# angelocatalani/neural-network-compression

Hardware: AMD Instinct MI355X
Metric: weights/sec through prune+k-means (K=256) (higher is better)
Workload: dtype f32

## Files before the change

### neural_network_compression_amd/csrc/nnc_sort.hip

```cpp
#include <hip/hip_runtime.h>
#include <cmath>
#include <cstdlib>
#include <cstring>

#include <algorithm>
#include <string>

#include "nnc.h"

extern "C" const char *nnc_last_error(void);
int nnc_set_error_(int code, const char *msg);

#ifndef OS_THREADS
#define OS_THREADS 1024
#endif
#define OS_WAVES (OS_THREADS / 64)
#ifndef OS_ITEMS
#define OS_ITEMS 16
#endif
#ifndef OS_BLOCKS_PER_CU
#define OS_BLOCKS_PER_CU 1
#endif
#ifndef OS_RANK_LDS
#define OS_RANK_LDS 1
#endif
#define OS_TILE (OS_THREADS * OS_ITEMS)
#define OS_MAXBITS 9
#define OS_MAXR (1 << OS_MAXBITS)
#define OS_MAXPASS 4
#define OS_SPIN_LIMIT (1 << 22)
#define OSP_THREADS 1024
#define OSP_PER 16
#define OSP_TILE (OSP_THREADS * OSP_PER)

__device__ __forceinline__ unsigned f32_ord(float v)
{
    const unsigned b = __float_as_uint(v);
    return (b & 0x80000000u) ? ~b : (b | 0x80000000u);
}
__device__ __forceinline__ float f32_unord(unsigned o)
{
    return __uint_as_float((o & 0x80000000u) ? (o ^ 0x80000000u) : ~o);
}

struct OsMap { unsigned lo_neg, hi_neg, lo_pos, hi_pos, span_neg; int bounded; };
struct OsPlan { int passes; int shift[OS_MAXPASS]; int rb[OS_MAXPASS]; };

__device__ __forceinline__ unsigned os_key(const OsMap &m, float e, bool &outside)
{
    const unsigned o = f32_ord(e);
    if (!m.bounded) return o;
    if (e < 0.0f) { outside |= (o < m.lo_neg) | (o > m.hi_neg); const unsigned c = o < m.lo_neg ? m.lo_neg : (o > m.hi_neg ? m.hi_neg : o); return c - m.lo_neg; }
    outside |= (o < m.lo_pos) | (o > m.hi_pos);
    const unsigned c = o < m.lo_pos ? m.lo_pos : (o > m.hi_pos ? m.hi_pos : o);
    return m.span_neg + (c - m.lo_pos);
}
__device__ __forceinline__ float os_value(const OsMap &m, unsigned k)
{
    if (!m.bounded) return f32_unord(k);
    return f32_unord(k < m.span_neg ? k + m.lo_neg : k - m.span_neg + m.lo_pos);
}

#define OS_CTRL_WORDS 4

template <bool SKIPZ>
__global__ __launch_bounds__(OSP_THREADS) void k_os_prep(const float *__restrict__ x, long long n, unsigned *__restrict__ keys,
                                                         unsigned long long *__restrict__ ctrl, long long cap, OsMap km, int rb0, unsigned *__restrict__ ghist)
{
    __shared__ unsigned comp_s[SKIPZ ? OSP_TILE : 1];
    __shared__ unsigned hist_s[OS_MAXR];
    __shared__ unsigned wave_tot[OSP_THREADS / 64];
    __shared__ unsigned long long base_s;
    const int tid = threadIdx.x, lane = tid & 63, wv = tid >> 6;
    for (int i = tid; i < OS_MAXR; i += OSP_THREADS) hist_s[i] = 0u;
    __syncthreads();
    const bool vec = (reinterpret_cast<uintptr_t>(x) & 15) == 0;
    const float4 *x4 = reinterpret_cast<const float4 *>(x);
    const unsigned mask0 = (1u << rb0) - 1u;
    bool outside = false;
    const long long ntiles = (n + OSP_TILE - 1) / OSP_TILE;
    auto load_tile = [&](long long tt, float (&e)[OSP_PER]) {
        const long long tile0 = tt * OSP_TILE;
        if (tt >= ntiles) return;
        if (vec && tile0 + OSP_TILE <= n) {
#pragma unroll
            for (int j = 0; j < OSP_PER / 4; j++) {
                const float4 q = x4[(tile0 >> 2) + (long long)j * OSP_THREADS + tid];
                e[4 * j] = q.x; e[4 * j + 1] = q.y; e[4 * j + 2] = q.z; e[4 * j + 3] = q.w;
            }
        } else {
#pragma unroll
            for (int j = 0; j < OSP_PER; j++) {
                const long long i = tile0 + (long long)j * OSP_THREADS + tid;
                e[j] = i < n ? x[i] : 0.0f;
            }
        }
    };
    float en[OSP_PER];
    load_tile(blockIdx.x, en);
    for (long long t = blockIdx.x; t < ntiles; t += gridDim.x) {
        const long long tile0 = t * OSP_TILE;
        const bool fast = vec && tile0 + OSP_TILE <= n;
        float e[OSP_PER];
#pragma unroll
        for (int j = 0; j < OSP_PER; j++) e[j] = en[j];
        load_tile(t + gridDim.x, en);
        unsigned key[OSP_PER];
        unsigned take = 0;
#pragma unroll
        for (int j = 0; j < OSP_PER; j++) {
            bool ok = SKIPZ ? !(e[j] == 0.0f) : true;
            if (!SKIPZ && !fast) ok = tile0 + (long long)j * OSP_THREADS + tid < n;
            key[j] = 0u;
            if (ok) { key[j] = os_key(km, e[j], outside); take |= 1u << j; }
        }
#pragma unroll
        for (int j = 0; j < OSP_PER; j++)
            if (take & (1u << j)) atomicAdd(&hist_s[key[j] & mask0], 1u);
        if (SKIPZ) {
            const unsigned c = (unsigned)__popc(take);
            unsigned sc = c;
            for (int off = 1; off < 64; off <<= 1) { const unsigned o = __shfl_up(sc, off); if (lane >= off) sc += o; }
            if (lane == 63) wave_tot[wv] = sc;
            __syncthreads();
            unsigned pre = 0, tot = 0;
            for (int w = 0; w < OSP_THREADS / 64; w++) { const unsigned o = wave_tot[w]; if (w < wv) pre += o; tot += o; }
            if (tid == 0) base_s = atomicAdd(ctrl, (unsigned long long)tot);
            unsigned at = pre + sc - c;
#pragma unroll
            for (int j = 0; j < OSP_PER; j++)
                if (take & (1u << j)) comp_s[at++] = key[j];
            __syncthreads();
            const long long base = (long long)base_s;
            for (unsigned i = tid; i < tot; i += OSP_THREADS)
                if (base + i < cap) keys[base + i] = comp_s[i];
            __syncthreads();
        }
    }
    if (outside) atomicOr(ctrl + 1, 1ull);
    __syncthreads();
    for (int i = tid; i < OS_MAXR; i += OSP_THREADS) {
        const unsigned v = hist_s[i];
        if (v) atomicAdd(&ghist[i], v);
    }
}

#ifdef NNC_DIAG
__device__ unsigned long long *g_os_trace = nullptr;
extern "C" int nnc_debug_os_trace(void *buf)
{
    unsigned long long *p = reinterpret_cast<unsigned long long *>(buf);
    return hipMemcpyToSymbol(HIP_SYMBOL(g_os_trace), &p, sizeof(p)) == hipSuccess ? NNC_OK : NNC_EHIP;
}
#define OS_STAMP(i) do { if (g_os_trace && t == 0) g_os_trace[((size_t)pass * 8192 + (size_t)(tile < 8192 ? tile : 8191)) * 8 + (i)] = __builtin_amdgcn_s_memrealtime(); } while (0)
#else
#define OS_STAMP(i) do { } while (0)
#endif

__device__ __forceinline__ void os_publish(unsigned long long *w, unsigned tag, unsigned v)
{
    __hip_atomic_store(w, ((unsigned long long)tag << 32) | v, __ATOMIC_RELAXED, __HIP_MEMORY_SCOPE_AGENT);
}
__device__ __forceinline__ unsigned long long os_peek(const unsigned long long *w)
{
    return __hip_atomic_load(w, __ATOMIC_RELAXED, __HIP_MEMORY_SCOPE_AGENT);
}

template <int RB, bool FULL>
__device__ __forceinline__ void os_peers(unsigned d, bool valid, unsigned &plo, unsigned &phi)
{
    const unsigned long long all = FULL ? ~0ull : __ballot(valid);
    plo = (unsigned)all; phi = (unsigned)(all >> 32);
#pragma unroll
    for (int b = 0; b < RB; b++) {
        const int m = ((int)(d << (31 - b))) >> 31;
        const unsigned long long mb = FULL ? __ballot(m != 0) : __ballot(valid && m != 0);
        plo &= ~((unsigned)mb ^ (unsigned)m);
        phi &= ~((unsigned)(mb >> 32) ^ (unsigned)m);
    }
}

#ifndef OS_LOOK
#define OS_LOOK 4
#endif

template <int RB, int SRC, int DST>
__global__ __launch_bounds__(OS_THREADS, OS_BLOCKS_PER_CU * OS_THREADS / 256) void k_os_pass(const void *__restrict__ in_, void *__restrict__ out_, long long n, int shift, int pass, int nrb,
                                                           const unsigned *__restrict__ ghist, unsigned *__restrict__ ghist_next, unsigned long long *__restrict__ status,
                                                           unsigned long long *__restrict__ ctrl, OsMap km, long long n_neg, long long n_zero, int abl)
{
    constexpr int R = 1 << RB;
    constexpr unsigned MASK = (unsigned)R - 1u;
    constexpr int DPT = (R + OS_THREADS - 1) / OS_THREADS;
    __shared__ unsigned keys_s[OS_TILE];
    __shared__ unsigned short wcnt[OS_WAVES][R];
    __shared__ unsigned short tpre[R];
    __shared__ unsigned gpos[R];
    __shared__ unsigned gdig[R];
    __shared__ unsigned nhist[OS_MAXR];
    __shared__ unsigned wsum[OS_WAVES];
    __shared__ long long tile_s;
    const int t = threadIdx.x, lane = t & 63, wv = t >> 6;
    const unsigned *in_k = reinterpret_cast<const unsigned *>(in_);
    const float *in_f = reinterpret_cast<const float *>(in_);
    unsigned *out_k = reinterpret_cast<unsigned *>(out_);
    float *out_f = reinterpret_cast<float *>(out_);
    const unsigned tagA = 2u * (unsigned)pass + 1u, tagP = tagA + 1u;
    unsigned *ticket = reinterpret_cast<unsigned *>(ctrl + 2) + pass;
    const int nshift = shift + RB;
    const unsigned nmask = nrb > 0 ? (1u << nrb) - 1u : 0u;
    {
        unsigned v[DPT], own = 0;
#pragma unroll
        for (int r = 0; r < DPT; r++) { const int d = t * DPT + r; v[r] = d < R ? ghist[d] : 0u; own += v[r]; }
        unsigned sc = own;
        for (int off = 1; off < 64; off <<= 1) { const unsigned o = __shfl_up(sc, off); if (lane >= off) sc += o; }
        if (lane == 63) wsum[wv] = sc;
        for (int i = t; i < OS_MAXR; i += OS_THREADS) nhist[i] = 0u;
        __syncthreads();
        unsigned run = sc - own;
        for (int w = 0; w < wv; w++) run += wsum[w];
#pragma unroll
        for (int r = 0; r < DPT; r++) { const int d = t * DPT + r; if (d < R) gdig[d] = run; run += v[r]; }
        __syncthreads();
    }
    const long long ntiles = (n + OS_TILE - 1) / OS_TILE;
    bool gave_up = false;
    for (;;) {
        if (t == 0) tile_s = (long long)atomicAdd(ticket, 1u);
        for (int d = t; d < R; d += OS_THREADS) {
#pragma unroll
            for (int w = 0; w < OS_WAVES; w++) wcnt[w][d] = 0;
        }
#if OS_RANK_LDS
        static_assert((size_t)OS_WAVES * R * 8 <= (size_t)OS_TILE * 4, "lane masks do not fit the tile buffer");
        for (int i = t; i < OS_WAVES * R * 2; i += OS_THREADS) keys_s[i] = 0u;
#endif
        __syncthreads();
        const long long tile = tile_s;
        if (tile >= ntiles) break;
        OS_STAMP(0);
        const long long tile0 = tile * OS_TILE;
        const int cnt_tile = (int)((n - tile0) < OS_TILE ? (n - tile0) : OS_TILE);
        const bool full = cnt_tile == OS_TILE;
        unsigned key[OS_ITEMS];
        unsigned short rnk[OS_ITEMS];
#pragma unroll
        for (int i = 0; i < OS_ITEMS; i++) {
            const int idx = wv * (64 * OS_ITEMS) + i * 64 + lane;
            if (SRC == 0) key[i] = (full || idx < cnt_tile) ? in_k[tile0 + idx] : 0xFFFFFFFFu;
            else key[i] = (full || idx < cnt_tile) ? f32_ord(in_f[tile0 + idx]) : 0xFFFFFFFFu;
        }
#ifdef NNC_DIAG
        if (g_os_trace) { if (key[OS_ITEMS - 1] == 0x12345678u && key[0] == 0x87654321u) keys_s[0] = 1u; OS_STAMP(1); }
#endif
        if (nrb > 0) {
#pragma unroll
            for (int i = 0; i < OS_ITEMS; i++) {
                const int idx = wv * (64 * OS_ITEMS) + i * 64 + lane;
                if ((full || idx < cnt_tile) && !(abl & 8)) atomicAdd(&nhist[(key[i] >> nshift) & nmask], 1u);
            }
        }
#pragma unroll
        for (int i = 0; i < OS_ITEMS; i++) {
            const int idx = wv * (64 * OS_ITEMS) + i * 64 + lane;
            const bool valid = full || idx < cnt_tile;
            const unsigned d = (key[i] >> shift) & MASK;
            unsigned plo, phi;
#if OS_RANK_LDS
            unsigned long long *mrow = reinterpret_cast<unsigned long long *>(keys_s) + wv * R;
            if (valid) atomicOr(&mrow[d], 1ull << lane);
            __builtin_amdgcn_wave_barrier();
            const unsigned long long pm = valid ? mrow[d] : 0ull;
            plo = (unsigned)pm; phi = (unsigned)(pm >> 32);
            if (abl & 2) { plo = lane < 32 ? 1u << lane : 0u; phi = lane >= 32 ? 1u << (lane - 32) : 0u; }
#else
            if (abl & 2) { plo = lane < 32 ? 1u << lane : 0u; phi = lane >= 32 ? 1u << (lane - 32) : 0u; }
            else if (full) os_peers<RB, true>(d, true, plo, phi);
            else os_peers<RB, false>(d, valid, plo, phi);
#endif
            const unsigned before = (unsigned)__builtin_amdgcn_mbcnt_hi(phi, __builtin_amdgcn_mbcnt_lo(plo, 0u));
            unsigned prev = 0;
            if (valid) {
                prev = wcnt[wv][d];
                if (before == 0) {
                    wcnt[wv][d] = (unsigned short)(prev + (unsigned)__popc(plo) + (unsigned)__popc(phi));
#if OS_RANK_LDS
                    mrow[d] = 0ull;
#endif
                }
            }
            rnk[i] = (unsigned short)(prev + before);
            __builtin_amdgcn_wave_barrier();
        }
        __syncthreads();
        OS_STAMP(2);
        unsigned tc[DPT], own = 0;
#pragma unroll
        for (int r = 0; r < DPT; r++) {
            const int d = t * DPT + r;
            tc[r] = 0;
            if (d < R) {
                unsigned run = 0;
#pragma unroll
                for (int w = 0; w < OS_WAVES; w++) { const unsigned c = wcnt[w][d]; wcnt[w][d] = (unsigned short)run; run += c; }
                tc[r] = run;
                os_publish(&status[(size_t)tile * R + d], tile == 0 ? tagP : tagA, run);
            }
            own += tc[r];
        }
        {
            unsigned sc = own;
            for (int off = 1; off < 64; off <<= 1) { const unsigned o = __shfl_up(sc, off); if (lane >= off) sc += o; }
            if (lane == 63) wsum[wv] = sc;
            __syncthreads();
            unsigned run = sc - own;
            for (int w = 0; w < wv; w++) run += wsum[w];
#pragma unroll
            for (int r = 0; r < DPT; r++) { const int d = t * DPT + r; if (d < R) tpre[d] = (unsigned short)run; run += tc[r]; }
        }
        __syncthreads();
#pragma unroll
        for (int i = 0; i < OS_ITEMS; i++) {
            const int idx = wv * (64 * OS_ITEMS) + i * 64 + lane;
            if (full || idx < cnt_tile) {
                const unsigned d = (key[i] >> shift) & MASK;
                keys_s[(unsigned)tpre[d] + (unsigned)wcnt[wv][d] + (unsigned)rnk[i]] = key[i];
            }
        }
        OS_STAMP(3);
        if (DST == 1 && n_zero > 0) {
            const long long per = ((n_zero + ntiles - 1) / ntiles + 3) & ~3ll;
            const long long z0 = tile * per, z1 = (z0 + per < n_zero) ? z0 + per : n_zero;
            float *zp = out_f + n_neg;
            if ((reinterpret_cast<uintptr_t>(zp) & 15) == 0) {
                for (long long i = z0 + 4ll * t; i + 3 < z1; i += 4ll * OS_THREADS) *reinterpret_cast<float4 *>(zp + i) = make_float4(0.f, 0.f, 0.f, 0.f);
                if (t == 0) for (long long i = z0 + ((z1 - z0) & ~3ll); i < z1; i++) zp[i] = 0.0f;
            } else {
                for (long long i = z0 + t; i < z1; i += OS_THREADS) zp[i] = 0.0f;
            }
        }
#pragma unroll
        for (int r = 0; r < DPT; r++) {
            const int d = t * DPT + r;
            if (d >= R) continue;
            unsigned excl = 0;
            if (tile > 0 && !(abl & 1)) {
                long long i = tile - 1;
                int polls = 0;
                bool done = false;
                while (!done) {
                    unsigned long long w[OS_LOOK];
#pragma unroll
                    for (int j = 0; j < OS_LOOK; j++) w[j] = (i - j >= 0) ? os_peek(&status[(size_t)(i - j) * R + d]) : 0ull;
                    int used = 0;
#pragma unroll
                    for (int j = 0; j < OS_LOOK; j++) {
                        if (!done && used == j) {
                            const unsigned tg = (unsigned)(w[j] >> 32);
                            if (tg == tagP) { excl += (unsigned)w[j]; done = true; }
                            else if (tg == tagA) { excl += (unsigned)w[j]; used = j + 1; }
                        }
                    }
                    if (!done) {
                        i -= used;
                        if (used == 0) {
                            if (++polls > OS_SPIN_LIMIT) { gave_up = true; done = true; }
                            __builtin_amdgcn_s_sleep(1);
                        } else polls = 0;
                    }
                }
                os_publish(&status[(size_t)tile * R + d], tagP, excl + tc[r]);
            }
            gpos[d] = gdig[d] + excl - (unsigned)tpre[d];
        }
        OS_STAMP(4);
        __syncthreads();
        OS_STAMP(5);
        for (int j = t; j < cnt_tile; j += OS_THREADS) {
            const unsigned kv = keys_s[j];
            const unsigned d = (kv >> shift) & MASK;
            const unsigned r = gpos[d] + (unsigned)j;
            if ((long long)r < n && !(abl & 4)) {
                if (DST == 0) out_k[r] = kv;
                else out_f[(long long)r + ((long long)r >= n_neg ? n_zero : 0)] = os_value(km, kv);
            }
        }
        OS_STAMP(6);
        __syncthreads();
        OS_STAMP(7);
    }
    if (gave_up) atomicOr(ctrl + 1, 2ull);
    if (nrb > 0) {
        for (int i = t; i <= (int)nmask; i += OS_THREADS) {
            const unsigned v = nhist[i];
            if (v) atomicAdd(&ghist_next[i], v);
        }
    }
}

static unsigned host_ord(float v)
{
    unsigned b;
    std::memcpy(&b, &v, 4);
    return (b & 0x80000000u) ? ~b : (b | 0x80000000u);
}

static size_t al256(size_t b) { return (b + 255) & ~(size_t)255; }

static int os_cus()
{
    static int cus[64] = {0};
    int dev = 0;
    if (hipGetDevice(&dev) != hipSuccess || dev < 0 || dev >= 64) return 256;
    if (!cus[dev]) {
        int v = 0;
        if (hipDeviceGetAttribute(&v, hipDeviceAttributeMultiprocessorCount, dev) != hipSuccess || v <= 0) v = 256;
        cus[dev] = v;
    }
    return cus[dev];
}

static OsPlan os_plan(int bits)
{
    OsPlan pl;
    std::memset(&pl, 0, sizeof(pl));
    int rb;
    if (bits <= 8) { pl.passes = 1; rb = 8; }
    else if (bits <= 16) { pl.passes = 2; rb = 8; }
    else if (bits <= 18) { pl.passes = 2; rb = 9; }
    else if (bits <= 24) { pl.passes = 3; rb = 8; }
    else if (bits <= 27) { pl.passes = 3; rb = 9; }
    else { pl.passes = 4; rb = 8; }
    for (int p = 0; p < pl.passes; p++) { pl.shift[p] = p * rb; pl.rb[p] = rb; }
    return pl;
}

static size_t os_status_bytes(int64_t n_keys)
{
    const int64_t ntiles = (n_keys + OS_TILE - 1) / OS_TILE;
    return al256((size_t)std::max<int64_t>(ntiles, 1) * OS_MAXR * 8);
}
static size_t os_ws_bytes(int64_t n_keys)
{
    return 2 * al256((size_t)n_keys * 4 + 16) + al256(OS_CTRL_WORDS * 8) + al256((size_t)(OS_MAXPASS + 1) * OS_MAXR * 4) + os_status_bytes(n_keys) + 256;
}
static unsigned char *os_ws_base(void *ws) { return reinterpret_cast<unsigned char *>((reinterpret_cast<uintptr_t>(ws) + 255) & ~(uintptr_t)255); }

static int os_sort(const float *x, int64_t n, bool skip_zeros, int64_t n_neg, int64_t n_zero, const OsMap &km, int bits, float *sorted_out, void *ws,
                   size_t ws_bytes, int32_t *flag_dev, const char *who, void *stream)
{
    const int64_t n_keys = skip_zeros ? n - n_zero : n;
    if (!ws || ws_bytes < os_ws_bytes(n_keys)) return nnc_set_error_(NNC_ENOSPACE, (std::string(who) + ": workspace too small").c_str());
    hipStream_t s = reinterpret_cast<hipStream_t>(stream);
    unsigned char *b = os_ws_base(ws);
    unsigned *ka = reinterpret_cast<unsigned *>(b); b += al256((size_t)n_keys * 4 + 16);
    unsigned *kb = reinterpret_cast<unsigned *>(b); b += al256((size_t)n_keys * 4 + 16);
    unsigned long long *ctrl = reinterpret_cast<unsigned long long *>(b); b += al256(OS_CTRL_WORDS * 8);
    unsigned *ghist = reinterpret_cast<unsigned *>(b); b += al256((size_t)(OS_MAXPASS + 1) * OS_MAXR * 4);
    unsigned long long *status = reinterpret_cast<unsigned long long *>(b);
    hipError_t e;
    const size_t zero_bytes = al256(OS_CTRL_WORDS * 8) + al256((size_t)(OS_MAXPASS + 1) * OS_MAXR * 4) + os_status_bytes(n_keys);
    if ((e = hipMemsetAsync(ctrl, 0, zero_bytes, s)) != hipSuccess) return nnc_set_error_(NNC_EHIP, hipGetErrorString(e));
    if (skip_zeros && n_zero > 0 && n_keys == 0 && (e = hipMemsetAsync(sorted_out + n_neg, 0, (size_t)n_zero * 4, s)) != hipSuccess) return nnc_set_error_(NNC_EHIP, hipGetErrorString(e));
    const OsPlan pl = os_plan(bits);
    int abl = 0;
#ifdef NNC_DIAG
    { const char *ev = getenv("NNC_OS_ABLATE"); abl = ev ? atoi(ev) : 0; }
#endif
    if (n_keys > 0) {
        const long long ptiles = (n + OSP_TILE - 1) / OSP_TILE;
        const int pgrid = (int)std::min<long long>(std::max<long long>(ptiles, 1), 2LL * os_cus());
        if (skip_zeros) hipLaunchKernelGGL((k_os_prep<true>), dim3(pgrid), dim3(OSP_THREADS), 0, s, x, (long long)n, ka, ctrl, (long long)n_keys, km, pl.rb[0], ghist);
        else hipLaunchKernelGGL((k_os_prep<false>), dim3(pgrid), dim3(OSP_THREADS), 0, s, x, (long long)n, (unsigned *)nullptr, ctrl, (long long)n_keys, km, pl.rb[0], ghist);
        if ((e = hipGetLastError()) != hipSuccess) return nnc_set_error_(NNC_EHIP, hipGetErrorString(e));
        const long long ntiles = (n_keys + OS_TILE - 1) / OS_TILE;
        const int grid = (int)std::min<long long>(ntiles, (long long)OS_BLOCKS_PER_CU * os_cus());
        const void *src = skip_zeros ? (const void *)ka : (const void *)x;
        unsigned *dst = skip_zeros ? kb : ka;
        for (int p = 0; p < pl.passes; p++) {
            const bool first_f = (p == 0 && !skip_zeros), last = (p == pl.passes - 1);
            void *o = last ? (void *)sorted_out : (void *)dst;
#define OS_LAUNCH(SRC, DST) do { \
                if (pl.rb[p] == 9) hipLaunchKernelGGL((k_os_pass<9, SRC, DST>), dim3(grid), dim3(OS_THREADS), 0, s, src, o, (long long)n_keys, pl.shift[p], p, last ? 0 : pl.rb[p + 1], \
                                                      ghist + (size_t)p * OS_MAXR, ghist + (size_t)(p + 1) * OS_MAXR, status, ctrl, km, (long long)(skip_zeros ? n_neg : n_keys), (long long)(skip_zeros ? n_zero : 0), abl); \
                else hipLaunchKernelGGL((k_os_pass<8, SRC, DST>), dim3(grid), dim3(OS_THREADS), 0, s, src, o, (long long)n_keys, pl.shift[p], p, last ? 0 : pl.rb[p + 1], \
                                        ghist + (size_t)p * OS_MAXR, ghist + (size_t)(p + 1) * OS_MAXR, status, ctrl, km, (long long)(skip_zeros ? n_neg : n_keys), (long long)(skip_zeros ? n_zero : 0), abl); \
            } while (0)
            if (first_f && last) OS_LAUNCH(1, 1);
            else if (first_f) OS_LAUNCH(1, 0);
            else if (last) OS_LAUNCH(0, 1);
            else OS_LAUNCH(0, 0);
#undef OS_LAUNCH
            if ((e = hipGetLastError()) != hipSuccess) return nnc_set_error_(NNC_EHIP, hipGetErrorString(e));
            src = dst;
            dst = (dst == ka) ? kb : ka;
        }
    }
    if (flag_dev && (e = hipMemcpyAsync(flag_dev, reinterpret_cast<unsigned char *>(ctrl) + 8, 4, hipMemcpyDeviceToDevice, s)) != hipSuccess)
        return nnc_set_error_(NNC_EHIP, hipGetErrorString(e));
    return NNC_OK;
}

static OsMap os_identity()
{
    OsMap m;
    std::memset(&m, 0, sizeof(m));
    return m;
}

extern "C" size_t nnc_sort_workspace_bytes(int64_t n) { return n <= 0 ? 0 : os_ws_bytes(n); }

extern "C" int nnc_sort_f32(const float *x, int64_t n, float *sorted_out, void *ws, size_t ws_bytes, void *stream)
{
    if (n < 0 || n >= ((int64_t)1 << 31) || (n > 0 && (!x || !sorted_out))) return nnc_set_error_(NNC_EINVAL, "nnc_sort_f32: bad argument");
    if (n == 0) return NNC_OK;
    return os_sort(x, n, false, 0, 0, os_identity(), 32, sorted_out, ws, ws_bytes, nullptr, "nnc_sort_f32", stream);
}

extern "C" size_t nnc_sort_pruned_workspace_bytes(int64_t n, int64_t n_neg, int64_t n_zero)
{
    if (n <= 0 || n_neg < 0 || n_zero < 0 || n_neg + n_zero > n) return 0;
    return os_ws_bytes(n - n_zero);
}

extern "C" int nnc_sort_pruned_f32(const float *x, int64_t n, int64_t n_neg, int64_t n_zero, float *sorted_out, void *ws,
                                   size_t ws_bytes, void *stream)
{
    if (n < 0 || n_neg < 0 || n_zero < 0 || n_neg + n_zero > n || n >= ((int64_t)1 << 31) || (n > 0 && (!x || !sorted_out)))
        return nnc_set_error_(NNC_EINVAL, "nnc_sort_pruned_f32: bad argument");
    if (n == 0) return NNC_OK;
    return os_sort(x, n, true, n_neg, n_zero, os_identity(), 32, sorted_out, ws, ws_bytes, nullptr, "nnc_sort_pruned_f32", stream);
}

static int rs_bounds(float vmin, float vmax, float thr, int64_t n_neg, int64_t n_pos, OsMap *bd)
{
    if (!(thr > 0.0f) || !std::isfinite(thr) || !std::isfinite(vmin) || !std::isfinite(vmax)) return 0;
    OsMap b;
    std::memset(&b, 0, sizeof(b));
    b.bounded = 1;
    unsigned long long total = 0;
    if (n_neg > 0) {
        if (!(vmin <= -thr)) return 0;
        b.lo_neg = host_ord(vmin); b.hi_neg = host_ord(-thr);
        b.span_neg = b.hi_neg - b.lo_neg + 1u;
        total += b.span_neg;
    }
    if (n_pos > 0) {
        if (!(vmax >= thr)) return 0;
        b.lo_pos = host_ord(thr); b.hi_pos = host_ord(vmax);
        total += (unsigned long long)(b.hi_pos - b.lo_pos) + 1ull;
    }
    if (total == 0 || total > (1ull << 27)) return 0;
    int bits = 1;
    while ((1ull << bits) < total) bits++;
    *bd = b;
    return bits;
}

extern "C" int32_t nnc_sort_pruned_bounded_bits(float vmin, float vmax, float thr, int64_t n_neg, int64_t n_pos)
{
    OsMap b;
    return rs_bounds(vmin, vmax, thr, n_neg, n_pos, &b);
}

extern "C" size_t nnc_sort_pruned_bounded_workspace_bytes(int64_t n_nz)
{
    if (n_nz < 0) return 0;
    return os_ws_bytes(n_nz);
}

int nnc_sort_pruned_bounded_flagged_(const float *x, int64_t n, int64_t n_neg, int64_t n_zero, float vmin, float vmax, float thr,
                                     float *sorted_out, void *ws, size_t ws_bytes, int32_t *flag_dev, void *stream);
extern "C" int nnc_sort_pruned_bounded_f32(const float *x, int64_t n, int64_t n_neg, int64_t n_zero, float vmin, float vmax, float thr,
                                           float *sorted_out, void *ws, size_t ws_bytes, void *stream)
{
    return nnc_sort_pruned_bounded_flagged_(x, n, n_neg, n_zero, vmin, vmax, thr, sorted_out, ws, ws_bytes, nullptr, stream);
}

extern "C" const int32_t *nnc_sort_pruned_bounded_flag(void *ws, int64_t n_nonzero)
{
    if (!ws || n_nonzero < 0) return nullptr;
    unsigned char *b = os_ws_base(ws) + 2 * al256((size_t)n_nonzero * 4 + 16);
    return reinterpret_cast<const int32_t *>(b + 8);
}

int nnc_sort_pruned_bounded_flagged_(const float *x, int64_t n, int64_t n_neg, int64_t n_zero, float vmin, float vmax, float thr,
                                     float *sorted_out, void *ws, size_t ws_bytes, int32_t *flag_dev, void *stream)
{
    if (n < 0 || n_neg < 0 || n_zero < 0 || n_neg + n_zero > n || n >= ((int64_t)1 << 31) || (n > 0 && (!x || !sorted_out)))
        return nnc_set_error_(NNC_EINVAL, "nnc_sort_pruned_bounded_f32: bad argument");
    if (n == 0) return NNC_OK;
    const int64_t n_pos = n - n_neg - n_zero, n_nz = n_neg + n_pos;
    OsMap bd;
    std::memset(&bd, 0, sizeof(bd));
    bd.bounded = 1;
    const int bits = n_nz > 0 ? rs_bounds(vmin, vmax, thr, n_neg, n_pos, &bd) : 1;
    if (bits == 0) return nnc_set_error_(NNC_EINVAL, "nnc_sort_pruned_bounded_f32: bounds do not apply (see nnc_sort_pruned_bounded_bits)");
    return os_sort(x, n, true, n_neg, n_zero, bd, bits, sorted_out, ws, ws_bytes, flag_dev, "nnc_sort_pruned_bounded_f32", stream);
}
```

Baseline: 10.03 billion.

## Replace multi-pass onesweep radix sort with bucket scatter plus per-bucket counting sort

For bounded key ranges, the multi-pass onesweep LSD radix sort is replaced by an MSD scheme. Keys are compacted and counted per chunk, column-scanned, and scattered into top-digit buckets. Each bucket is then finished with an LDS counting sort on the low 14 bits, which also writes the zero fill and maps keys back to floats. This cuts the number of passes over the keys and avoids the decoupled-lookback chain. In exchange it adds more kernel launches, a per-chunk count matrix in the workspace, and is sensitive to skewed bucket sizes.

```diff
diff --git a/neural_network_compression_amd/csrc/nnc_sort.hip b/neural_network_compression_amd/csrc/nnc_sort.hip
--- a/neural_network_compression_amd/csrc/nnc_sort.hip
+++ b/neural_network_compression_amd/csrc/nnc_sort.hip
@@ -63,16 +63,16 @@
 
 #define OS_CTRL_WORDS 4
 
-template <bool SKIPZ>
+template <bool SKIPZ, int HR>
 __global__ __launch_bounds__(OSP_THREADS) void k_os_prep(const float *__restrict__ x, long long n, unsigned *__restrict__ keys,
                                                          unsigned long long *__restrict__ ctrl, long long cap, OsMap km, int rb0, unsigned *__restrict__ ghist)
 {
     __shared__ unsigned comp_s[SKIPZ ? OSP_TILE : 1];
-    __shared__ unsigned hist_s[OS_MAXR];
+    __shared__ unsigned hist_s[HR > 0 ? HR : 1];
     __shared__ unsigned wave_tot[OSP_THREADS / 64];
     __shared__ unsigned long long base_s;
     const int tid = threadIdx.x, lane = tid & 63, wv = tid >> 6;
-    for (int i = tid; i < OS_MAXR; i += OSP_THREADS) hist_s[i] = 0u;
+    for (int i = tid; i < HR; i += OSP_THREADS) hist_s[i] = 0u;
     __syncthreads();
     const bool vec = (reinterpret_cast<uintptr_t>(x) & 15) == 0;
     const float4 *x4 = reinterpret_cast<const float4 *>(x);
@@ -116,7 +116,7 @@
         }
 #pragma unroll
         for (int j = 0; j < OSP_PER; j++)
-            if (take & (1u << j)) atomicAdd(&hist_s[key[j] & mask0], 1u);
+            if (HR > 0 && (take & (1u << j))) atomicAdd(&hist_s[key[j] & mask0], 1u);
         if (SKIPZ) {
             const unsigned c = (unsigned)__popc(take);
             unsigned sc = c;
@@ -139,7 +139,7 @@
     }
     if (outside) atomicOr(ctrl + 1, 1ull);
     __syncthreads();
-    for (int i = tid; i < OS_MAXR; i += OSP_THREADS) {
+    for (int i = tid; i < HR; i += OSP_THREADS) {
         const unsigned v = hist_s[i];
         if (v) atomicAdd(&ghist[i], v);
     }
@@ -399,6 +399,234 @@
     }
 }
 
+#ifndef OSB_LBITS
+#define OSB_LBITS 14
+#endif
+#define OSB_THREADS 1024
+#ifndef OSB_ITEMS
+#define OSB_ITEMS 16
+#endif
+#define OSB_CHUNK (OSB_THREADS * OSB_ITEMS)
+#define OSB_MAXR0 (1 << (27 - OSB_LBITS))
+#define OSB_HEAVY 64
+#define OSB_HMAX 256
+
+static inline void osb_digits(int bits, int &d0, int &lb)
+{
+    d0 = std::max(bits - OSB_LBITS, std::min(bits, 11));
+    lb = bits - d0;
+}
+
+__device__ __forceinline__ void osb_scan_totals(const unsigned *__restrict__ ghist, int nb, unsigned *bst, unsigned *wsum)
+{
+    constexpr int PER = OSB_MAXR0 / OSB_THREADS;
+    const int t = threadIdx.x, lane = t & 63, wv = t >> 6;
+    unsigned v[PER], own = 0;
+#pragma unroll
+    for (int r = 0; r < PER; r++) { const int d = t * PER + r; v[r] = d < nb ? ghist[d] : 0u; own += v[r]; }
+    unsigned sc = own;
+    for (int off = 1; off < 64; off <<= 1) { const unsigned o = __shfl_up(sc, off); if (lane >= off) sc += o; }
+    if (lane == 63) wsum[wv] = sc;
+    __syncthreads();
+    unsigned run = sc - own;
+    for (int w = 0; w < wv; w++) run += wsum[w];
+#pragma unroll
+    for (int r = 0; r < PER; r++) { const int d = t * PER + r; if (d <= nb) bst[d] = run; run += v[r]; }
+    if (t * PER + PER == nb) bst[nb] = run;
+    __syncthreads();
+}
+
+__global__ __launch_bounds__(OSB_THREADS) void k_os_count(const unsigned *__restrict__ ka, long long n_keys, unsigned *__restrict__ cmat, int d0, int lb)
+{
+    __shared__ unsigned cnt[OSB_MAXR0];
+    const int t = threadIdx.x, nb = 1 << d0;
+    const unsigned dmask = (unsigned)nb - 1u;
+    for (int d = t; d < nb; d += OSB_THREADS) cnt[d] = 0u;
+    const long long c0 = (long long)blockIdx.x * OSB_CHUNK;
+    const int cn = (int)std::min<long long>(OSB_CHUNK, n_keys - c0);
+    unsigned key[OSB_ITEMS];
+#pragma unroll
+    for (int j = 0; j < OSB_ITEMS; j++) { const int i = j * OSB_THREADS + t; key[j] = i < cn ? ka[c0 + i] : 0u; }
+    __syncthreads();
+#pragma unroll
+    for (int j = 0; j < OSB_ITEMS; j++) if (j * OSB_THREADS + t < cn) atomicAdd(&cnt[(key[j] >> lb) & dmask], 1u);
+    __syncthreads();
+    unsigned *row = cmat + (size_t)blockIdx.x * nb;
+    for (int d = t; d < nb; d += OSB_THREADS) row[d] = cnt[d];
+}
+
+#define OSB_SCAN_ROWS 16
+__global__ __launch_bounds__(OSB_THREADS) void k_os_colscan(unsigned *__restrict__ cmat, long long rows, unsigned *__restrict__ tot, int d0)
+{
+    __shared__ unsigned part[OSB_THREADS / 64][64];
+    const int t = threadIdx.x, lane = t & 63, wv = t >> 6, nb = 1 << d0;
+    const int col = blockIdx.x * 64 + lane;
+    unsigned carry = 0;
+    for (long long blk = 0; blk < rows; blk += (long long)(OSB_THREADS / 64) * OSB_SCAN_ROWS) {
+        const long long r0 = blk + (long long)wv * OSB_SCAN_ROWS;
+        const int nr = col < nb ? (int)std::max<long long>(0, std::min<long long>(OSB_SCAN_ROWS, rows - r0)) : 0;
+        unsigned *cp = cmat + (size_t)std::min<long long>(r0, rows) * nb + col;
+        unsigned v[OSB_SCAN_ROWS], sum = 0;
+#pragma unroll
+        for (int i = 0; i < OSB_SCAN_ROWS; i++) { v[i] = i < nr ? cp[(unsigned)(i * nb)] : 0u; sum += v[i]; }
+        part[wv][lane] = sum;
+        __syncthreads();
+        unsigned run = carry, all = carry;
+        for (int w = 0; w < OSB_THREADS / 64; w++) { const unsigned p = part[w][lane]; if (w < wv) run += p; all += p; }
+#pragma unroll
+        for (int i = 0; i < OSB_SCAN_ROWS; i++) { if (i < nr) cp[(unsigned)(i * nb)] = run; run += v[i]; }
+        carry = all;
+        __syncthreads();
+    }
+    if (wv == 0 && col < nb) tot[col] = carry;
+}
+
+__global__ __launch_bounds__(OSB_THREADS) void k_os_scatter(const unsigned *__restrict__ ka, unsigned *__restrict__ kb, long long n_keys, const unsigned *__restrict__ tot,
+                                                            const unsigned *__restrict__ cmat, unsigned *__restrict__ bstart, int d0, int lb)
+{
+    __shared__ unsigned keys_s[OSB_CHUNK];
+    __shared__ unsigned gpos[OSB_MAXR0 + 1];
+    __shared__ unsigned cnt[OSB_MAXR0];
+    __shared__ unsigned short tpre[OSB_MAXR0];
+    __shared__ unsigned wsum[OSB_THREADS / 64];
+    const int t = threadIdx.x, lane = t & 63, wv = t >> 6, nb = 1 << d0;
+    const unsigned dmask = (unsigned)nb - 1u;
+    for (int d = t; d < nb; d += OSB_THREADS) cnt[d] = 0u;
+    const long long c0 = (long long)blockIdx.x * OSB_CHUNK;
+    const int cn = (int)std::min<long long>(OSB_CHUNK, n_keys - c0);
+    const unsigned *row = cmat + (size_t)blockIdx.x * nb;
+    unsigned key[OSB_ITEMS], rnk[OSB_ITEMS];
+#pragma unroll
+    for (int j = 0; j < OSB_ITEMS; j++) {
+        const int i = j * OSB_THREADS + t;
+        key[j] = i < cn ? ka[c0 + i] : 0u;
+    }
+    osb_scan_totals(tot, nb, gpos, wsum);
+    if (blockIdx.x == 0)
+        for (int d = t; d <= nb; d += OSB_THREADS) bstart[d] = gpos[d];
+#pragma unroll
+    for (int j = 0; j < OSB_ITEMS; j++) rnk[j] = j * OSB_THREADS + t < cn ? atomicAdd(&cnt[(key[j] >> lb) & dmask], 1u) : 0u;
+    __syncthreads();
+    {
+        constexpr int PER = OSB_MAXR0 / OSB_THREADS;
+        unsigned c[PER], above[PER], own = 0;
+#pragma unroll
+        for (int r = 0; r < PER; r++) { const int d = t * PER + r; c[r] = d < nb ? cnt[d] : 0u; above[r] = d < nb ? row[d] : 0u; own += c[r]; }
+        unsigned sc = own;
+        for (int off = 1; off < 64; off <<= 1) { const unsigned o = __shfl_up(sc, off); if (lane >= off) sc += o; }
+        __syncthreads();
+        if (lane == 63) wsum[wv] = sc;
+        __syncthreads();
+        unsigned run = sc - own;
+        for (int w = 0; w < wv; w++) run += wsum[w];
+#pragma unroll
+        for (int r = 0; r < PER; r++) {
+            const int d = t * PER + r;
+            if (d < nb) { tpre[d] = (unsigned short)run; gpos[d] = gpos[d] + above[r] - run; }
+            run += c[r];
+        }
+    }
+    __syncthreads();
+#pragma unroll
+    for (int j = 0; j < OSB_ITEMS; j++)
+        if (j * OSB_THREADS + t < cn) keys_s[(unsigned)tpre[(key[j] >> lb) & dmask] + rnk[j]] = key[j];
+    __syncthreads();
+    for (int j = t; j < cn; j += OSB_THREADS) {
+        const unsigned k = keys_s[j];
+        const unsigned p = gpos[(k >> lb) & dmask] + (unsigned)j;
+        if ((long long)p < n_keys) kb[p] = k;
+    }
+}
+
+__global__ __launch_bounds__(OSB_THREADS) void k_os_bucket(const unsigned *__restrict__ kb, float *__restrict__ out, long long n_keys, const unsigned *__restrict__ bstart,
+                                                           int d0, int lb, OsMap km, long long n_neg, long long n_zero)
+{
+    constexpr int PER = (1 << OSB_LBITS) / OSB_THREADS;
+    __shared__ uint4 h4[(1 << OSB_LBITS) / 4];
+    __shared__ unsigned wsum[OSB_THREADS / 64];
+    __shared__ unsigned hv_s[OSB_HMAX], hp_s[OSB_HMAX], hc_s[OSB_HMAX];
+    __shared__ unsigned nheavy;
+    unsigned *h = reinterpret_cast<unsigned *>(h4);
+    const int t = threadIdx.x, lane = t & 63, wv = t >> 6, d = blockIdx.x, nb = 1 << d0;
+    if (n_zero > 0) {
+        const long long per = ((n_zero + nb - 1) / nb + 3) & ~3ll;
+        const long long z0 = (long long)d * per, z1 = (z0 + per < n_zero) ? z0 + per : n_zero;
+        float *zp = out + n_neg;
+        if ((reinterpret_cast<uintptr_t>(zp) & 15) == 0) {
+            for (long long i = z0 + 4ll * t; i + 3 < z1; i += 4ll * OSB_THREADS) *reinterpret_cast<float4 *>(zp + i) = make_float4(0.f, 0.f, 0.f, 0.f);
+            if (t == 0) for (long long i = (z0 < z1 ? z0 + ((z1 - z0) & ~3ll) : z1); i < z1; i++) zp[i] = 0.0f;
+        } else {
+            for (long long i = z0 + t; i < z1; i += OSB_THREADS) zp[i] = 0.0f;
+        }
+    }
+    const long long s = std::min<long long>(bstart[d], n_keys), e = std::min<long long>(bstart[d + 1], n_keys);
+    if (e <= s) return;
+    const unsigned m = (unsigned)(e - s);
+    const unsigned *kp = kb + s;
+    const unsigned lmask = (1u << lb) - 1u, hi = (unsigned)d << lb;
+    auto put = [&](unsigned r, unsigned v) {
+        const long long g = s + (long long)r;
+        if (g < n_keys) out[g + (g >= n_neg ? n_zero : 0)] = os_value(km, hi | v);
+    };
+    if (m == 1) { if (t == 0) put(0, kp[0] & lmask); return; }
+#pragma unroll
+    for (int i = 0; i < PER / 4; i++) h4[i * OSB_THREADS + t] = make_uint4(0u, 0u, 0u, 0u);
+    if (t == 0) nheavy = 0u;
+    __syncthreads();
+    for (unsigned i0 = 0; i0 < m; i0 += 4u * OSB_THREADS) {
+        unsigned v[4];
+#pragma unroll
+        for (int j = 0; j < 4; j++) { const unsigned i = i0 + (unsigned)j * OSB_THREADS + t; v[j] = i < m ? (kp[i] & lmask) : 0xFFFFFFFFu; }
+#pragma unroll
+        for (int j = 0; j < 4; j++) {
+            if (v[j] == 0xFFFFFFFFu) continue;
+            const unsigned long long act = __ballot(1), same = __ballot(v[j] == (unsigned)__builtin_amdgcn_readfirstlane(v[j]));
+            if (same == act) { if (lane == __ffsll((long long)act) - 1) atomicAdd(&h[v[j]], (unsigned)__popcll(act)); }
+            else atomicAdd(&h[v[j]], 1u);
+        }
+    }
+    __syncthreads();
+    unsigned c[PER], own = 0;
+#pragma unroll
+    for (int i = 0; i < PER / 4; i++) {
+        const uint4 q = h4[t * (PER / 4) + i];
+        c[4 * i] = q.x; c[4 * i + 1] = q.y; c[4 * i + 2] = q.z; c[4 * i + 3] = q.w;
+    }
+#pragma unroll
+    for (int i = 0; i < PER; i++) own += c[i];
+    unsigned sc = own;
+    for (int off = 1; off < 64; off <<= 1) { const unsigned o = __shfl_up(sc, off); if (lane >= off) sc += o; }
+    if (lane == 63) wsum[wv] = sc;
+    __syncthreads();
+    unsigned run = sc - own;
+    for (int w = 0; w < wv; w++) run += wsum[w];
+    const bool in_lds = m <= (1u << OSB_LBITS);
+    const unsigned v0 = (unsigned)t * PER;
+#pragma unroll
+    for (int i = 0; i < PER; i++) {
+        const unsigned ci = c[i];
+        if (ci == 0) continue;
+        if (ci >= OSB_HEAVY) {
+            const unsigned q = atomicAdd(&nheavy, 1u);
+            if (q < OSB_HMAX) { hv_s[q] = v0 + i; hp_s[q] = run; hc_s[q] = ci; run += ci; continue; }
+        }
+        if (in_lds) for (unsigned k = 0; k < ci; k++) h[run + k] = v0 + i;
+        else for (unsigned k = 0; k < ci; k++) put(run + k, v0 + i);
+        run += ci;
+    }
+    __syncthreads();
+    const unsigned nh = std::min<unsigned>(nheavy, OSB_HMAX);
+    for (unsigned q = 0; q < nh; q++) {
+        const unsigned v = hv_s[q], p = hp_s[q], cq = hc_s[q];
+        if (in_lds) for (unsigned k = t; k < cq; k += OSB_THREADS) h[p + k] = v;
+        else for (unsigned k = t; k < cq; k += OSB_THREADS) put(p + k, v);
+    }
+    if (in_lds) {
+        __syncthreads();
+        for (unsigned j = t; j < m; j += OSB_THREADS) put(j, h[j]);
+    }
+}
+
 static unsigned host_ord(float v)
 {
     unsigned b;
@@ -445,12 +673,57 @@
 {
     return 2 * al256((size_t)n_keys * 4 + 16) + al256(OS_CTRL_WORDS * 8) + al256((size_t)(OS_MAXPASS + 1) * OS_MAXR * 4) + os_status_bytes(n_keys) + 256;
 }
+#define OSB_CNT_BYTES al256((size_t)2 * (OSB_MAXR0 + 1) * 4)
+static int64_t osb_chunks(int64_t n_keys) { return (n_keys + OSB_CHUNK - 1) / OSB_CHUNK; }
+static size_t osb_ws_bytes(int64_t n_keys)
+{
+    return 2 * al256((size_t)n_keys * 4 + 16) + al256(OS_CTRL_WORDS * 8) + OSB_CNT_BYTES + al256((size_t)osb_chunks(n_keys) * OSB_MAXR0 * 4) + 256;
+}
 static unsigned char *os_ws_base(void *ws) { return reinterpret_cast<unsigned char *>((reinterpret_cast<uintptr_t>(ws) + 255) & ~(uintptr_t)255); }
+
+static int osb_sort(const float *x, int64_t n, int64_t n_neg, int64_t n_zero, const OsMap &km, int bits, float *sorted_out, void *ws, size_t ws_bytes,
+                    int32_t *flag_dev, const char *who, void *stream)
+{
+    const int64_t n_keys = n - n_zero;
+    if (!ws || ws_bytes < osb_ws_bytes(n_keys)) return nnc_set_error_(NNC_ENOSPACE, (std::string(who) + ": workspace too small").c_str());
+    hipStream_t s = reinterpret_cast<hipStream_t>(stream);
+    unsigned char *b = os_ws_base(ws);
+    unsigned *ka = reinterpret_cast<unsigned *>(b); b += al256((size_t)n_keys * 4 + 16);
+    unsigned *kb = reinterpret_cast<unsigned *>(b); b += al256((size_t)n_keys * 4 + 16);
+    unsigned long long *ctrl = reinterpret_cast<unsigned long long *>(b); b += al256(OS_CTRL_WORDS * 8);
+    unsigned *tot = reinterpret_cast<unsigned *>(b), *bstart = tot + (OSB_MAXR0 + 1); b += OSB_CNT_BYTES;
+    unsigned *cmat = reinterpret_cast<unsigned *>(b);
+    hipError_t e;
+    if ((e = hipMemsetAsync(ctrl, 0, al256(OS_CTRL_WORDS * 8), s)) != hipSuccess) return nnc_set_error_(NNC_EHIP, hipGetErrorString(e));
+    if (n_keys == 0) {
+        if (n_zero > 0 && (e = hipMemsetAsync(sorted_out + n_neg, 0, (size_t)n_zero * 4, s)) != hipSuccess) return nnc_set_error_(NNC_EHIP, hipGetErrorString(e));
+    } else {
+        int d0, lb;
+        osb_digits(bits, d0, lb);
+        const long long ptiles = (n + OSP_TILE - 1) / OSP_TILE;
+        const int pgrid = (int)std::min<long long>(std::max<long long>(ptiles, 1), 2LL * os_cus());
+        const long long chunks = osb_chunks(n_keys);
+        hipLaunchKernelGGL((k_os_prep<true, 0>), dim3(pgrid), dim3(OSP_THREADS), 0, s, x, (long long)n, ka, ctrl, (long long)n_keys, km, 1, (unsigned *)nullptr);
+        if ((e = hipGetLastError()) != hipSuccess) return nnc_set_error_(NNC_EHIP, hipGetErrorString(e));
+        hipLaunchKernelGGL(k_os_count, dim3((unsigned)chunks), dim3(OSB_THREADS), 0, s, ka, (long long)n_keys, cmat, d0, lb);
+        if ((e = hipGetLastError()) != hipSuccess) return nnc_set_error_(NNC_EHIP, hipGetErrorString(e));
+        hipLaunchKernelGGL(k_os_colscan, dim3((1u << d0) + 63 >> 6), dim3(OSB_THREADS), 0, s, cmat, chunks, tot, d0);
+        if ((e = hipGetLastError()) != hipSuccess) return nnc_set_error_(NNC_EHIP, hipGetErrorString(e));
+        hipLaunchKernelGGL(k_os_scatter, dim3((unsigned)chunks), dim3(OSB_THREADS), 0, s, ka, kb, (long long)n_keys, tot, cmat, bstart, d0, lb);
+        if ((e = hipGetLastError()) != hipSuccess) return nnc_set_error_(NNC_EHIP, hipGetErrorString(e));
+        hipLaunchKernelGGL(k_os_bucket, dim3(1u << d0), dim3(OSB_THREADS), 0, s, kb, sorted_out, (long long)n_keys, bstart, d0, lb, km, (long long)n_neg, (long long)n_zero);
+        if ((e = hipGetLastError()) != hipSuccess) return nnc_set_error_(NNC_EHIP, hipGetErrorString(e));
+    }
+    if (flag_dev && (e = hipMemcpyAsync(flag_dev, reinterpret_cast<unsigned char *>(ctrl) + 8, 4, hipMemcpyDeviceToDevice, s)) != hipSuccess)
+        return nnc_set_error_(NNC_EHIP, hipGetErrorString(e));
+    return NNC_OK;
+}
 
 static int os_sort(const float *x, int64_t n, bool skip_zeros, int64_t n_neg, int64_t n_zero, const OsMap &km, int bits, float *sorted_out, void *ws,
                    size_t ws_bytes, int32_t *flag_dev, const char *who, void *stream)
 {
     const int64_t n_keys = skip_zeros ? n - n_zero : n;
+    if (km.bounded) return osb_sort(x, n, n_neg, n_zero, km, bits, sorted_out, ws, ws_bytes, flag_dev, who, stream);
     if (!ws || ws_bytes < os_ws_bytes(n_keys)) return nnc_set_error_(NNC_ENOSPACE, (std::string(who) + ": workspace too small").c_str());
     hipStream_t s = reinterpret_cast<hipStream_t>(stream);
     unsigned char *b = os_ws_base(ws);
@@ -471,8 +744,8 @@
     if (n_keys > 0) {
         const long long ptiles = (n + OSP_TILE - 1) / OSP_TILE;
         const int pgrid = (int)std::min<long long>(std::max<long long>(ptiles, 1), 2LL * os_cus());
-        if (skip_zeros) hipLaunchKernelGGL((k_os_prep<true>), dim3(pgrid), dim3(OSP_THREADS), 0, s, x, (long long)n, ka, ctrl, (long long)n_keys, km, pl.rb[0], ghist);
-        else hipLaunchKernelGGL((k_os_prep<false>), dim3(pgrid), dim3(OSP_THREADS), 0, s, x, (long long)n, (unsigned *)nullptr, ctrl, (long long)n_keys, km, pl.rb[0], ghist);
+        if (skip_zeros) hipLaunchKernelGGL((k_os_prep<true, OS_MAXR>), dim3(pgrid), dim3(OSP_THREADS), 0, s, x, (long long)n, ka, ctrl, (long long)n_keys, km, pl.rb[0], ghist);
+        else hipLaunchKernelGGL((k_os_prep<false, OS_MAXR>), dim3(pgrid), dim3(OSP_THREADS), 0, s, x, (long long)n, (unsigned *)nullptr, ctrl, (long long)n_keys, km, pl.rb[0], ghist);
         if ((e = hipGetLastError()) != hipSuccess) return nnc_set_error_(NNC_EHIP, hipGetErrorString(e));
         const long long ntiles = (n_keys + OS_TILE - 1) / OS_TILE;
         const int grid = (int)std::min<long long>(ntiles, (long long)OS_BLOCKS_PER_CU * os_cus());
@@ -567,7 +840,7 @@
 extern "C" size_t nnc_sort_pruned_bounded_workspace_bytes(int64_t n_nz)
 {
     if (n_nz < 0) return 0;
-    return os_ws_bytes(n_nz);
+    return osb_ws_bytes(n_nz);
 }
 
 int nnc_sort_pruned_bounded_flagged_(const float *x, int64_t n, int64_t n_neg, int64_t n_zero, float vmin, float vmax, float thr,
```

Result: no change. 10.09 billion (median of 6 runs) (+0.5%).
